# akvas/grates

Hardware: AMD Instinct MI355X
Metric: d/o-96 solutions/s to 0.25deg grid + full-cov GFLOP/s at 1/2/4/8 MI355X (higher is better)
Workload: dtype f64; 1 GPU; batch of 240 monthly solutions d/o 96 -> 0.25 deg GeographicGrid (720x1440), kernel ewh, per GPU; max_degree=96, epochs_per_gpu=240, parallelism=epochs sharded over 1 GPU(s), no collective, fused_kernel=True, fourfold_symmetry=True, rotation_folded_kernel=True, rotations=10, settle_launches=300

## Files before the change

grates_amd/_lib.py:

```python

import ctypes
import os

_HERE = os.path.dirname(os.path.abspath(__file__))
LIB_PATH = os.path.join(_HERE, 'lib', 'libshg.so')

c_double_p = ctypes.c_void_p
c_plan_p = ctypes.c_void_p


class ShgError(RuntimeError):

    def __init__(self, function, status, message):
        super().__init__('{0} failed with status {1}: {2}'.format(function, status, message))
        self.function = function
        self.status = status


PROTOTYPES = {
    'shg_plan_create': [ctypes.POINTER(c_plan_p), ctypes.c_int, ctypes.c_int, c_double_p, c_double_p, ctypes.c_int, c_double_p, ctypes.c_int],
    'shg_plan_destroy': [c_plan_p],
    'shg_plan_set_chunk': [c_plan_p, ctypes.c_int],
    'shg_plan_set_path': [c_plan_p, ctypes.c_int],
    'shg_plan_set_rotations': [c_plan_p, ctypes.c_int],
    'shg_plan_set_stage_limit': [c_plan_p, ctypes.c_int],
    'shg_plan_set_order_pruning': [c_plan_p, ctypes.c_int],
    'shg_plan_order_cutoffs': [c_plan_p, ctypes.POINTER(ctypes.c_int), ctypes.c_int, ctypes.POINTER(ctypes.c_int), ctypes.POINTER(ctypes.c_int)],
    'shg_rot_order_cutoffs': [ctypes.c_int, ctypes.c_int, c_double_p, c_double_p, ctypes.POINTER(ctypes.c_int), ctypes.c_int, ctypes.POINTER(ctypes.c_int)],
    'shg_rot_level_tables': [ctypes.c_int, ctypes.c_int, ctypes.c_int, ctypes.c_int, ctypes.c_int, c_double_p, ctypes.POINTER(ctypes.c_int32), c_double_p,
                             ctypes.c_int64, ctypes.POINTER(ctypes.c_int32), ctypes.c_int64],
    'shg_plan_info': [c_plan_p, ctypes.POINTER(ctypes.c_int64)],
    'shg_analysis_info': [c_plan_p, c_double_p],
    'shg_plan_profile': [c_plan_p, ctypes.c_int],
    'shg_plan_profile_read': [c_plan_p, ctypes.POINTER(ctypes.c_double), ctypes.POINTER(ctypes.c_int64)],
    'shg_synthesis': [c_plan_p, c_double_p, ctypes.c_int, c_double_p, ctypes.c_void_p],
    'shg_synthesis_points': [ctypes.c_int, c_double_p, c_double_p, c_double_p, ctypes.c_int, c_double_p, ctypes.c_int, c_double_p, ctypes.c_void_p],
    'shg_legendre': [ctypes.c_int, c_double_p, ctypes.c_int, c_double_p, ctypes.c_void_p],
    'shg_legendre_order': [ctypes.c_int, ctypes.c_int, c_double_p, ctypes.c_int, c_double_p, ctypes.c_void_p],
    'shg_trigonometric': [ctypes.c_int, c_double_p, ctypes.c_int, c_double_p, ctypes.c_void_p],
    'shg_synthesis_matrix_order': [ctypes.c_int, ctypes.c_int, ctypes.c_int, c_double_p, ctypes.c_int, c_double_p, ctypes.c_int, c_double_p, ctypes.c_int,
                                   c_double_p, c_double_p, ctypes.c_void_p],
# ... 138 lines not shown
```

grates_amd/csrc/common.h:

```cpp
#pragma once

#include <hip/hip_runtime.h>

#include <algorithm>
#include <atomic>
#include <cstdarg>
#include <cstdint>
#include <cstdio>
#include <cstdlib>
#include <mutex>
#include <vector>

#include "../../include/shg.h"

namespace shg {

int fail(int code, const char* fmt, ...);
int zero_fill(double* p, long long ld, long long cols, long long rows, hipStream_t stream);
int zero_fill(int* p, hipStream_t stream);
int triangle_copy(int n, const double* src, int ld, long long stride, int batch, double* dst, bool upper, hipStream_t stream);
enum ScratchSlot { kScratchSplitK = 0, kScratchAnaFold = 1, kScratchAnaTransform = 2, kScratchAnaSolution = 3, kScratchAnaFlag = 4,
                   kScratchSeriesIn = 5, kScratchSeriesOut = 6 ,
                   kScratchTriangle = 7 ,
                   kScratchBlocks = 8  };
// ... 207 lines not shown
constexpr int kRotPruneMaxDegree = 128;
constexpr int kEpochTile = 8;
constexpr int kLatTile = 64;

}

struct shg_plan {
    int device = 0;
    int N = 0, nlat = 0, nlon = 0;
    int ldlat = 0;
    bool sym4 = false;
    int rotR = 0;
    std::vector<double> lon_host;
    shg::DeviceArray<double> rot_trig;
    bool order_pruning = true;
    std::vector<int> rot_levels;
    std::vector<int> rot_level_set;
    std::vector<int> rot_trig_piece;
    std::vector<int> rot_item_rec, rot_item_nrec, rot_item_ntrip;
    shg::DeviceArray<int> rot_levtab_d;
    bool rot_levtab_valid = false;
    bool sym_ns = false;
    int ngroups = 1;
    int goff[5] = {0, 0, 0, 0, 0};
    int K = 0;
    int ncol = 0;
    int ncoltiles = 0;
    int chunk = 16;

    shg::DeviceArray<double> ct;
// ... 119 lines not shown
```

grates_amd/csrc/plan.hip:

```cpp
#include <cmath>
#include <cstring>
#include <string>

#include <map>
#include <memory>
#include <mutex>
#include <utility>
#include <vector>

#include "common.h"

namespace shg {

static thread_local std::string g_last_error;

int fail(int code, const char* fmt, ...) {
    char buf[512];
    va_list ap;
    va_start(ap, fmt);
    vsnprintf(buf, sizeof(buf), fmt, ap);
    va_end(ap);
    g_last_error = buf;
    return code;
}
// ... 478 lines not shown

extern "C" int shg_plan_set_stage_limit(shg_plan* p, int limit) {
    SHG_REQUIRE(p != nullptr, "shg_plan_set_stage_limit: NULL plan");
    std::unique_lock<std::mutex> lock(p->mtx);
    return rot_set_stage_limit(p, limit);
}

extern "C" int shg_plan_set_order_pruning(shg_plan* p, int enable) {
    SHG_REQUIRE(p != nullptr, "shg_plan_set_order_pruning: NULL plan");
    SHG_REQUIRE(enable == 0 || enable == 1, "shg_plan_set_order_pruning: %d not in {0, 1}", enable);
    std::unique_lock<std::mutex> lock(p->mtx);
    p->order_pruning = enable != 0;
    return SHG_OK;
}

extern "C" int shg_plan_order_cutoffs(const shg_plan* p, int* levels, int capacity, int* nblocks, int* enabled) {
    SHG_REQUIRE(p != nullptr && nblocks != nullptr, "shg_plan_order_cutoffs: NULL argument");
    SHG_REQUIRE(capacity >= 0 && (levels != nullptr || capacity == 0), "shg_plan_order_cutoffs: NULL table of %d entries", capacity);
    const bool applies = rot_applicable(p) && !p->rot_levels.empty();
    *nblocks = applies ? (int)p->rot_levels.size() : 0;
    if (enabled) *enabled = applies && p->order_pruning ? 1 : 0;
    for (int i = 0; i < *nblocks && i < capacity; ++i) levels[i] = p->rot_levels[i];
    return SHG_OK;
}

extern "C" int shg_rot_order_cutoffs(int N, int nlat, const double* colat_h, const double* kn_h, int* levels, int capacity, int* nblocks) {
    SHG_REQUIRE(N >= 1 && N <= kRotPruneMaxDegree, "shg_rot_order_cutoffs: degree %d out of range [1, %d]", N, kRotPruneMaxDegree);
    SHG_REQUIRE(nlat > 0 && colat_h && kn_h && nblocks, "shg_rot_order_cutoffs: NULL or empty table");
    SHG_REQUIRE(capacity >= 0 && (levels != nullptr || capacity == 0), "shg_rot_order_cutoffs: NULL table of %d entries", capacity);
    std::vector<int> badmap, lv;
// ... 55 lines not shown
        return fail(SHG_ERR_UNSUPPORTED, "shg_plan_set_rotations: the panel of %d rotations at degree %d does not fit the LDS", want, p->N);
    }
    SHG_HIP(hipDeviceSynchronize());
    if (rot_applicable(p)) {
        const int rc = build_rot_trig(p, p->lon_host.data());
        if (rc) return rc;
    }
    return SHG_OK;
}

extern "C" int shg_plan_info(const shg_plan* p, int64_t which[8]) {
    SHG_REQUIRE(p != nullptr && which != nullptr, "shg_plan_info: NULL argument");
    which[0] = p->N;
    which[1] = p->nlat;
    which[2] = p->nlon;
    which[3] = (p->sym4 ? 1 : 0) | (p->sym_ns ? 2 : 0) | (rot_applicable(p) ? 4 : 0);
    which[4] = p->chunk;
    which[5] = p->K;
    which[6] = (p->path >= 2 || (p->path == 0 && (rot_applicable(p) || fused_chunk_for(p) != 0 || fused32_applicable(p)))) ? 1 : 0;
    which[7] = p->path | (rot_applicable(p) ? p->rotR << 8 : 0);
    return SHG_OK;
}
```

grates_amd/csrc/synthesis_rot.hip:

```cpp
#include <algorithm>
#include <cmath>
#include <cstdlib>

#include "common.h"

#ifndef SHG_STORE_AUX
#define SHG_STORE_AUX 2
#endif

namespace shg {

typedef double double4_t __attribute__((ext_vector_type(4)));
typedef double double2_t __attribute__((ext_vector_type(2)));
typedef unsigned int uint4_t __attribute__((ext_vector_type(4)));

#ifndef SHG_ROT_PREFERENCE
#define SHG_ROT_PREFERENCE 10, 9, 6, 3
#endif
#ifndef SHG_ROT_WAVES
#define SHG_ROT_WAVES 8
#endif
#ifndef SHG_RING_DEPTH
#define SHG_RING_DEPTH (SHG_ROT_WAVES > 8 ? 3 : 5)
#endif
// ... 2 lines not shown
constexpr int kRingDepth = SHG_RING_DEPTH;
constexpr int kRingSlots = kRingDepth + 1;
constexpr int kRingDoubles = kWaves * kRingSlots * 128;
constexpr int kMaxClasses = kRotMaxClasses;

template <int R>
struct RotTraits {
    static constexpr int kClasses = R / 2 + 1, kTwo = R % 2 == 0 ? 2 : 1, kAcc = 2 * R;
    static constexpr int acc_of(int r) { return r == 0 ? 0 : (R % 2 == 0 && 2 * r == R) ? 2 : 2 * kTwo + 4 * (r - 1); }
};

struct RotParams {
    int N, nlat, nlon, B, nit, nh;
    int nd;
    int nct;
    int npieces;
    int cls_nk[kMaxClasses];
    int cls_cnt[kMaxClasses];
    int nslot;
#ifdef SHG_EXPERIMENT
    int dbg;
    int stagger;
    int stagger2;
#endif
    int Qtot;
    const double* cpk4;
    const double* pkf;
    const int4* itemtab;
    int nrec, ntrip;
    int* sem;
// ... 37 lines not shown

__device__ __forceinline__ void store_b64_soff(double v, int4_s rsrc, unsigned voff, unsigned soff) {
    asm volatile("s_mov_b32 m0, %3\n\ts_nop 0\n\tbuffer_store_dwordx2 %0, %1, %2, m0 offen nt"
                 :
                 : "v"(v), "v"(voff), "s"(rsrc), "s"(soff)
                 : "memory");
}

template <int N>
__device__ __forceinline__ void wait_vmcnt() {
    asm volatile("s_waitcnt vmcnt(%0)" ::"i"(N) : "memory");
    __builtin_amdgcn_sched_barrier(0);
}

template <int R>
__device__ __forceinline__ void rot_images(double4_t* acc, int r);

template <>
__device__ __forceinline__ void rot_images<6>(double4_t* acc, int r) {
    constexpr double g = 0.86602540378443864676;
    const double ca0 = acc[0][r], sb0 = acc[1][r], ca3 = acc[2][r], sb3 = acc[3][r];
    const double ca1 = acc[4][r], sa1 = acc[5][r], cb1 = acc[6][r], sb1 = acc[7][r];
    const double ca2 = acc[8][r], sa2 = acc[9][r], cb2 = acc[10][r], sb2 = acc[11][r];
#pragma unroll
    for (int sgn = 0; sgn < 2; ++sgn) {
        const double x0 = sgn ? ca0 - sb0 : ca0 + sb0, x3 = sgn ? ca3 - sb3 : ca3 + sb3;
        const double x1 = sgn ? ca1 - sb1 : ca1 + sb1, y1 = sgn ? cb1 + sa1 : cb1 - sa1;
        const double x2 = sgn ? ca2 - sb2 : ca2 + sb2, y2 = sgn ? cb2 + sa2 : cb2 - sa2;
        const double t = fma(-0.5, x2, x0);
        const double e0 = x0 + x2, e1 = fma(g, y2, t), e2 = fma(-g, y2, t);
        const double u = fma(0.5, x1, -x3);
        const double o0 = x1 + x3, o1 = fma(g, y1, u), o2 = fma(g, y1, -u);
        acc[6 * sgn + 0][r] = e0 + o0;
        acc[6 * sgn + 3][r] = e0 - o0;
        acc[6 * sgn + 1][r] = e1 + o1;
        acc[6 * sgn + 4][r] = e1 - o1;
        acc[6 * sgn + 2][r] = e2 + o2;
        acc[6 * sgn + 5][r] = e2 - o2;
    }
}

template <>
__device__ __forceinline__ void rot_images<3>(double4_t* acc, int r) {
    constexpr double g = 0.86602540378443864676;
    const double ca0 = acc[0][r], sb0 = acc[1][r];
    const double ca1 = acc[2][r], sa1 = acc[3][r], cb1 = acc[4][r], sb1 = acc[5][r];
#pragma unroll
    for (int sgn = 0; sgn < 2; ++sgn) {
        const double x0 = sgn ? ca0 - sb0 : ca0 + sb0;
        const double x1 = sgn ? ca1 - sb1 : ca1 + sb1, y1 = sgn ? cb1 + sa1 : cb1 - sa1;
        const double t = fma(-0.5, x1, x0);
        acc[3 * sgn + 0][r] = x0 + x1;
        acc[3 * sgn + 1][r] = fma(g, y1, t);
        acc[3 * sgn + 2][r] = fma(-g, y1, t);
    }
}

template <>
__device__ __forceinline__ void rot_images<9>(double4_t* acc, int r) {
    constexpr double c1 = 0.76604444311897803520, c2 = 0.17364817766693034885, c4 = -0.93969262078590838405;
    constexpr double s1 = 0.64278760968653932632, s2 = 0.98480775301220805937, s3 = 0.86602540378443864676, s4 = 0.34202014332566873304;
    const double ca0 = acc[0][r], sb0 = acc[1][r];
    double ca[4], sa[4], cb[4], sb[4];
#pragma unroll
    for (int j = 0; j < 4; ++j) {
        ca[j] = acc[2 + 4 * j][r];
        sa[j] = acc[3 + 4 * j][r];
        cb[j] = acc[4 + 4 * j][r];
        sb[j] = acc[5 + 4 * j][r];
    }
#pragma unroll
    for (int sgn = 0; sgn < 2; ++sgn) {
        const double x0 = sgn ? ca0 - sb0 : ca0 + sb0;
        double x[4], y[4];
#pragma unroll
        for (int j = 0; j < 4; ++j) {
            x[j] = sgn ? ca[j] - sb[j] : ca[j] + sb[j];
            y[j] = sgn ? cb[j] + sa[j] : cb[j] - sa[j];
        }
        const double x1 = x[0], x2 = x[1], x3 = x[2], x4 = x[3], y1 = y[0], y2 = y[1], y3 = y[2], y4 = y[3];
        const double t = (x1 + x2) + x4, x03 = x0 + x3;
        const double h = fma(-0.5, x3, x0), u = s3 * y3;
        const double C1 = fma(c1, x1, fma(c2, x2, fma(c4, x4, h)));
        const double C2 = fma(c2, x1, fma(c4, x2, fma(c1, x4, h)));
        const double C3 = fma(-0.5, t, x03);
        const double C4 = fma(c4, x1, fma(c1, x2, fma(c2, x4, h)));
        const double S1 = fma(s1, y1, fma(s2, y2, fma(s4, y4, u)));
        const double S2 = fma(s2, y1, fma(s4, y2, fma(-s1, y4, -u)));
        const double S3 = s3 * ((y1 - y2) + y4);
        const double S4 = fma(s4, y1, fma(-s1, y2, fma(-s2, y4, u)));
        acc[9 * sgn + 0][r] = x03 + t;
        acc[9 * sgn + 1][r] = C1 + S1;
        acc[9 * sgn + 8][r] = C1 - S1;
        acc[9 * sgn + 2][r] = C2 + S2;
        acc[9 * sgn + 7][r] = C2 - S2;
        acc[9 * sgn + 3][r] = C3 + S3;
        acc[9 * sgn + 6][r] = C3 - S3;
        acc[9 * sgn + 4][r] = C4 + S4;
        acc[9 * sgn + 5][r] = C4 - S4;
    }
}

template <>
__device__ __forceinline__ void rot_images<10>(double4_t* acc, int r) {
    constexpr double c1 = 0.80901699437494742410, c2 = 0.30901699437494742410;
    constexpr double s1 = 0.58778525229247312917, s2 = 0.95105651629515357212;
    const double ca0 = acc[0][r], sb0 = acc[1][r], ca5 = acc[2][r], sb5 = acc[3][r];
    double ca[4], sa[4], cb[4], sb[4];
#pragma unroll
    for (int j = 0; j < 4; ++j) {
        ca[j] = acc[4 + 4 * j][r];
        sa[j] = acc[5 + 4 * j][r];
        cb[j] = acc[6 + 4 * j][r];
        sb[j] = acc[7 + 4 * j][r];
    }
#pragma unroll
    for (int sgn = 0; sgn < 2; ++sgn) {
        const double x0 = sgn ? ca0 - sb0 : ca0 + sb0, x5 = sgn ? ca5 - sb5 : ca5 + sb5;
        double x[4], y[4];
#pragma unroll
        for (int j = 0; j < 4; ++j) {
            x[j] = sgn ? ca[j] - sb[j] : ca[j] + sb[j];
            y[j] = sgn ? cb[j] + sa[j] : cb[j] - sa[j];
        }
        const double x1 = x[0], x2 = x[1], x3 = x[2], x4 = x[3], y1 = y[0], y2 = y[1], y3 = y[2], y4 = y[3];
        const double e0 = (x0 + x2) + x4;
        const double a1 = fma(c2, x2, fma(-c1, x4, x0)), b1 = fma(s2, y2, s1 * y4);
        const double a2 = fma(-c1, x2, fma(c2, x4, x0)), b2 = fma(s1, y2, -(s2 * y4));
        const double e1 = a1 + b1, e4 = a1 - b1, e2 = a2 + b2, e3 = a2 - b2;
        const double o0 = (x1 + x3) + x5;
        const double p = fma(c1, x1, fma(-c2, x3, -x5)), q = fma(s1, y1, s2 * y3);
        const double u = fma(c2, x1, fma(-c1, x3, x5)), v = fma(s2, y1, -(s1 * y3));
        const double o1 = q + p, o4 = q - p, o2 = v + u, o3 = v - u;
        acc[10 * sgn + 0][r] = e0 + o0;
        acc[10 * sgn + 5][r] = e0 - o0;
        acc[10 * sgn + 1][r] = e1 + o1;
        acc[10 * sgn + 6][r] = e1 - o1;
        acc[10 * sgn + 2][r] = e2 + o2;
        acc[10 * sgn + 7][r] = e2 - o2;
        acc[10 * sgn + 3][r] = e3 + o3;
        acc[10 * sgn + 8][r] = e3 - o3;
        acc[10 * sgn + 4][r] = e4 + o4;
        acc[10 * sgn + 9][r] = e4 - o4;
    }
}

struct RotStream {
    const double* iptr;
    const double* ibase;
    const double* ifirst;
    const double* ilast;
    int irem;
    unsigned im0, ring_lds;
    int cslot, pf;
    double2_t tx, abx;
};

constexpr int EP = 4;
__device__ __forceinline__ void rot_stream_init(RotStream& S, const RotParams& P, const double* As, int wave) {
    const unsigned lds0 = (unsigned)(size_t)(__attribute__((address_space(3))) const void*)As;
    S.ring_lds = lds0 + (unsigned)wave * (kRingSlots * 1024);
    S.im0 = S.ring_lds;
    const int ct0 = min(wave / EP, P.nct - 1);
    const int nq = (P.nct - ct0 + kColStride - 1) / kColStride;
    S.ifirst = P.trig + (size_t)ct0 * P.npieces * 128;
    S.ilast = S.ifirst + (size_t)(nq - 1) * kColStride * P.npieces * 128;
    S.ibase = S.ifirst;
    S.iptr = S.ifirst;
    S.irem = P.npieces;
    S.cslot = 0;
    S.pf = 0;
    S.tx = (double2_t){0.0, 0.0};
    S.abx = (double2_t){0.0, 0.0};
}

__device__ __forceinline__ void rot_issue_piece(RotStream& S, const RotParams& P, unsigned lane_off) {
    glds16(S.iptr, lane_off, S.im0);
#if defined(SHG_ROT_X) && (SHG_ROT_X & 1)
    return;
// ... 50 lines not shown
    acc[A0] = __builtin_amdgcn_mfma_f64_16x16x4f64(AB_.x, T_.x, acc[A0], 0, 0, 0);                        \
    ROT_PRIO(2);                                                                                          \
    acc[A0 + 1] = __builtin_amdgcn_mfma_f64_16x16x4f64(AB_.x, T_.y, acc[A0 + 1], 0, 0, 0);                \
    acc[A0 + 2] = __builtin_amdgcn_mfma_f64_16x16x4f64(AB_.y, T_.x, acc[A0 + 2], 0, 0, 0);                \
    acc[A0 + 3] = __builtin_amdgcn_mfma_f64_16x16x4f64(AB_.y, T_.y, acc[A0 + 3], 0, 0, 0);                \
    ROT_PRIO(0)
#define ROT_MFMA2_FIRST(A0, T_, AB_)                                                                      \
    acc[A0] = (A0) == 0 ? __builtin_amdgcn_mfma_f64_16x16x4f64(AB_.x, T_.x, acc[A0], 0, 0, 0)              \
                        : __builtin_amdgcn_mfma_f64_16x16x4f64(AB_.x, T_.x, kZero4, 0, 0, 0);             \
    acc[A0 + 1] = __builtin_amdgcn_mfma_f64_16x16x4f64(AB_.y, T_.y, kZero4, 0, 0, 0)
#define ROT_MFMA4_FIRST(A0, T_, AB_)                                                                      \
    acc[A0] = __builtin_amdgcn_mfma_f64_16x16x4f64(AB_.x, T_.x, kZero4, 0, 0, 0);                         \
    acc[A0 + 1] = __builtin_amdgcn_mfma_f64_16x16x4f64(AB_.x, T_.y, kZero4, 0, 0, 0);                     \
    acc[A0 + 2] = __builtin_amdgcn_mfma_f64_16x16x4f64(AB_.y, T_.x, kZero4, 0, 0, 0);                     \
    acc[A0 + 3] = __builtin_amdgcn_mfma_f64_16x16x4f64(AB_.y, T_.y, kZero4, 0, 0, 0)
#define ROT_CLASS(C, MF, A0, NACC)                                                                        \
    {                                                                                                     \
        const int nk_ = P.cls_nk[C];                                                                      \
        int i_ = 0;                                                                                       \
        if (nk_ >= 2) {                                                                                   \
            ROT_FETCH(ty, aby);                                                                           \
            MF##_FIRST(A0, tx, abx);                                                                      \
            ROT_FETCH(tx, abx);                                                                           \
            MF(A0, ty, aby);                                                                              \
            i_ = 2;                                                                                       \
        } else if (nk_ == 1) {                                                                            \
            ROT_FETCH(ty, aby);                                                                           \
            MF##_FIRST(A0, tx, abx);                                                                      \
            tx = ty;                                                                                      \
            abx = aby;                                                                                    \
            i_ = 1;                                                                                       \
        } else {                                                                                          \
            _Pragma("unroll") for (int z_ = ((A0) == 0 ? 1 : 0); z_ < (NACC); ++z_) acc[(A0) + z_] = kZero4; \
        }                                                                                                 \
        for (; i_ + 2 <= nk_; i_ += 2) {                                                                  \
            ROT_FETCH(ty, aby);                                                                           \
            MF(A0, tx, abx);                                                                              \
            ROT_FETCH(tx, abx);                                                                           \
            MF(A0, ty, aby);                                                                              \
        }                                                                                                 \
        if (i_ < nk_) {                                                                                   \
            ROT_FETCH(ty, aby);                                                                           \
            MF(A0, tx, abx);                                                                              \
            tx = ty;                                                                                      \
            abx = aby;                                                                                    \
        }                                                                                                 \
    }
    const double4_t kZero4 = {0.0, 0.0, 0.0, 0.0};
    double2_t tx = S.tx, abx = S.abx, ty = {0.0, 0.0}, aby = {0.0, 0.0};
    const int ct0 = wave / EP;
    for (int ct = ct0, q = 0; ct < P.nct; ct += kColStride, ++q) {
        (void)q;
        double4_t acc[T::kAcc];
        {
            const double2_t* z = panel + P.nslot * PR + rt * 16 + fk;
#pragma unroll
            for (int r = 0; r < 4; ++r) acc[0][r] = z[4 * r].x;
        }
#pragma unroll
        for (int c = 0; c < T::kClasses; ++c) {
            if (c < T::kTwo) {
                ROT_CLASS(c, ROT_MFMA2, 2 * c, 2)
            } else {
                ROT_CLASS(c, ROT_MFMA4, 2 * T::kTwo + 4 * (c - T::kTwo), 4)
            }
        }
// ... 19 lines not shown
                int w = n2 + k * nR - (ascending ? 0 : P.nd);
                w = w >= P.nlon ? w - P.nlon : w;
                const int soff = (ascending ? w + 16 * ct : w + P.nd - 16 * ct - 16) * 8;
                double a_lo, a_hi, b_lo, b_hi;
                pair_exchange(acc[t][0], acc[t][2], 0xAAAAAAAAAAAAAAAAull, a_lo, a_hi);
                pair_exchange(acc[t][1], acc[t][3], 0xAAAAAAAAAAAAAAAAull, b_lo, b_hi);
                const double2_t va = ascending ? (double2_t){a_lo, a_hi} : (double2_t){a_hi, a_lo};
                const double2_t vb = ascending ? (double2_t){b_lo, b_hi} : (double2_t){b_hi, b_lo};
                const unsigned lane_col = (ascending ? asc : desc) + (unsigned)soff;
                __builtin_amdgcn_raw_buffer_store_b128(__builtin_bit_cast(uint4_t, va), rsrc, row_a + lane_col, 0, SHG_STORE_AUX);
                __builtin_amdgcn_raw_buffer_store_b128(__builtin_bit_cast(uint4_t, vb), rsrc, row_b + lane_col, 0, SHG_STORE_AUX);
            }
        }
        ROT_STAMP(4 + 2 * min(q, 3));
    }
    S.tx = tx;
    S.abx = abx;
#undef ROT_CLASS
#undef ROT_MFMA2
#undef ROT_MFMA4
#undef ROT_MFMA2_FIRST
#undef ROT_MFMA4_FIRST
#undef ROT_FETCH
}

__device__ __forceinline__ void panel_put(double2_t* panel, int index, double2_t v) { panel[index] = v; }

template <bool NS, typename PanelPtr>
__device__ __forceinline__ void rot_phase1(const RotParams& P, PanelPtr panel, const int4* recs_wave, int bt, int it, int lane) {
    const int fr = lane & 15, fk = lane >> 4;
    constexpr int ASTRIDE = NS ? 128 : 64;
    typedef int int4_v __attribute__((ext_vector_type(4)));
    typedef const int4_v __attribute__((address_space(4))) crec_t;
// ... 175 lines not shown
        if (tid == 0) legendre_token_acquire(P.sem, P.sem_limit);
        __syncthreads();
    }
    if (!SHG_DBG(P, 2)) rot_phase1<NS>(P, panel, P.itemtab + (size_t)wave * P.nrec, bt, it, lane);
    ROT_STAMP(1);
    __syncthreads();
    if (P.sem_limit > 0 && tid == 0) legendre_token_release(P.sem);
    ROT_STAMP(2);
#ifdef SHG_EXPERIMENT
    if (P.stagger2 > 0 && wave >= EP) {
        const long long t0 = wall_clock64();
        for (int i = 0; i < 100000 && (long long)wall_clock64() - t0 < P.stagger2; ++i) __builtin_amdgcn_s_sleep(4);
    }
#endif

    if (wave / EP < P.nct && !SHG_DBG(P, 4)) {
        const double2_t* const ringp = reinterpret_cast<const double2_t*>(As) + wave * (kRingSlots * 64) + lane;
        rot_issue_piece(S, P, (unsigned)lane * 16u);
        wait_vmcnt<kRingDepth>();
        S.tx = ringp[0];
        S.cslot = 1;
        S.abx = panel[(wave % EP) * 16 + fr + fk * PR];
        S.pf = P.npieces > 1 ? 1 : 0;
        rot_phase2<NS, R>(P, As, panel, S, wave, lane, bt * 4, it);
        wait_vmcnt<4 * R>();
    } else {
        wait_vmcnt<0>();
    }
    ROT_STAMP(12);
}



static inline void order_class(int R, int m, int& cls, int& sign) {
    const int rho = m % R;
    const int r = 2 * rho <= R ? rho : R - rho;
    sign = 2 * rho <= R ? 1 : -1;
    if (R % 2 == 0)
        cls = r == 0 ? 0 : 2 * r == R ? 1 : r + 1;
    else
// ... 96 lines not shown
                const double arg = (double)m * lon_h[nlon / 2 + c];
                double* dst = &tab[(((size_t)ct * npieces + ks) * 64 + l) * 2];
                dst[0] = std::cos(arg);
                dst[1] = sg * std::sin(arg);
            }
}

int build_rot_trig(shg_plan* p, const double* lon_h) {
    const std::vector<int> full(1, p->N);
    const std::vector<int>& levels = p->rot_level_set.empty() ? full : p->rot_level_set;
    std::vector<double> all, tab;
    p->rot_trig_piece.clear();
    for (int level : levels) {
        rot_trig_stream(p->rotR, p->N, level, p->nlon, lon_h, tab);
        p->rot_trig_piece.push_back((int)(all.size() / 128));
        all.insert(all.end(), tab.begin(), tab.end());
    }
    p->rot_levtab_valid = false;
    return upload(p->rot_trig, all);
}

constexpr double kRotPruneTau = 1e-30;
constexpr int kRotLevelStep = 10;

void rot_order_cutoffs(int N, int nlat, const double* colat, const double* kn, bool ns, std::vector<int>& levels) {
    const int nh = nlat / 2;
    const int nit = ns ? ceil_div(nh, 8) : ceil_div(nlat, 16);
    levels.assign(nit, 0);
    std::vector<double> a, b, big(N + 1);
    recursion_tables(N, a, b);
// ... 86 lines not shown
    int rc = build_pkf_table(p, ns, R, stream);
    if (rc) return rc;
    const int nbt = ceil_div(B, 4);
    const int nit = ns ? ceil_div(p->nlat / 2, 8) : ceil_div(p->nlat, 16);
    rc = pack_coefficients_fused(p, ns, R, anm, B, stream);
    if (rc) return rc;
    RotParams P;
    P.N = p->N;
    P.nlat = p->nlat;
    P.nlon = p->nlon;
    P.B = B;
    P.nit = nit;
    P.nh = p->nlat / 2;
    P.nd = p->nlon / (2 * R);
    P.nct = ceil_div(P.nd, 16);
    P.nslot = rot_layout(R, p->N, P.cls_nk, P.cls_cnt, nullptr);
    P.npieces = P.nslot / 4;
#ifdef SHG_EXPERIMENT
    P.dbg = experiment_switches();
    P.stagger = getenv("SHG_STAGGER") ? atoi(getenv("SHG_STAGGER")) : 0;
    P.stagger2 = getenv("SHG_STAGGER2") ? atoi(getenv("SHG_STAGGER2")) : 0;
#endif
    P.Qtot = p->Qtot;
    P.cpk4 = p->cpk4.get();
    P.pkf = p->pkf.get();
    P.itemtab = reinterpret_cast<const int4*>(p->itemtab_d.get());
    P.nrec = p->itemtab_nrec;
    P.ntrip = p->itemtab_ntrip;
    P.sem = p->sem_d.get();
    P.sem_limit = p->sem_d ? p->stage_limit : 0;
// ... 51 lines not shown
```

grates_amd/engine.py:

```python

import ctypes
import hashlib

import numpy as np

from . import _lib


def _torch():
    import torch
    return torch


def require_gpu():
    torch = _torch()
    if not torch.cuda.is_available():
        raise RuntimeError('grates_amd: no GPU visible -- the hot path runs on MI355X only (there is no CPU fallback)')
    _lib.load()
    return torch


def device(index=None):
    torch = require_gpu()
    return torch.device('cuda', torch.cuda.current_device() if index is None else index)
# ... 45 lines not shown
        if handle is not None and handle.value:
            try:
                _lib.load().shg_plan_destroy(handle)
            except Exception:
                pass
            self._handle = None

    def info(self):
        arr = (ctypes.c_int64 * 8)()
        _lib.call('shg_plan_info', self._handle, arr)
        nblocks, enabled = ctypes.c_int(0), ctypes.c_int(0)
        _lib.call('shg_plan_order_cutoffs', self._handle, None, 0, ctypes.byref(nblocks), ctypes.byref(enabled))
        levels = (ctypes.c_int * max(nblocks.value, 1))()
        _lib.call('shg_plan_order_cutoffs', self._handle, levels, nblocks.value, ctypes.byref(nblocks), ctypes.byref(enabled))
        return {'max_degree': arr[0], 'nlat': arr[1], 'nlon': arr[2], 'fourfold_symmetry': bool(arr[3] & 1), 'north_south_symmetry': bool(arr[3] & 2),
                'rotation_symmetry': bool(arr[3] & 4), 'epochs_per_pass': arr[4], 'k_slots': arr[5], 'fused': bool(arr[6]), 'path': int(arr[7]) & 0xff, 'rotations': int(arr[7]) >> 8,
                'order_pruning': bool(enabled.value), 'order_cutoffs': [int(levels[i]) for i in range(nblocks.value)]}

    def set_path(self, path):
        _lib.call('shg_plan_set_path', self._handle, {'auto': 0, 'staged': 1, 'fused': 2, 'fused32': 5, 'rot': 6}[path])

    def set_stage_limit(self, limit):
        _lib.call('shg_plan_set_stage_limit', self._handle, int(limit))

    def set_order_pruning(self, enable):
        _lib.call('shg_plan_set_order_pruning', self._handle, 1 if enable else 0)

    def set_rotations(self, R):
        _lib.call('shg_plan_set_rotations', self._handle, int(R))

    def set_chunk(self, epochs_per_pass):
        _lib.call('shg_plan_set_chunk', self._handle, int(epochs_per_pass))

    PROFILE_KINDS = ('pack_coefficients', 'legendre_stage', 'lon_stage', 'covprop', 'analysis_lon', 'analysis_solve', 'k6', 'k7')

    def profile(self, enable=True, kinds=None):
        if enable and kinds:
            mask = 0
            for name in kinds:
                mask |= 1 << (self.PROFILE_KINDS.index(name) + 1)
            _lib.call('shg_plan_profile', self._handle, mask)
# ... 1163 lines not shown
```

include/shg.h:

```cpp
#ifndef SHG_H
#define SHG_H

#include <stdint.h>

#ifdef __cplusplus
extern "C" {
#endif

typedef struct shg_plan shg_plan;

typedef enum {
    SHG_OK = 0,
    SHG_ERR_INVALID = -1,
    SHG_ERR_HIP = -2,
    SHG_ERR_NOMEM = -3,
    SHG_ERR_UNSUPPORTED = -4
} shg_status;

int shg_plan_create(shg_plan** out, int N, int nlat, const double* colat_h, const double* kn_h,
                    int nlon, const double* lon_h, int device);
int shg_plan_destroy(shg_plan* plan);

int shg_plan_set_chunk(shg_plan* plan, int epochs_per_pass);

int shg_plan_set_path(shg_plan* plan, int path);

int shg_plan_set_stage_limit(shg_plan* plan, int limit);

int shg_plan_set_rotations(shg_plan* plan, int R);

int shg_plan_set_order_pruning(shg_plan* plan, int enable);
int shg_plan_order_cutoffs(const shg_plan* plan, int* levels, int capacity, int* nblocks, int* enabled);
int shg_rot_order_cutoffs(int N, int nlat, const double* colat_h, const double* kn_h, int* levels, int capacity, int* nblocks);
int shg_rot_level_tables(int R, int N, int level, int ns, int nlon, const double* lon_h, int32_t header[24], double* trig,
                         int64_t trig_capacity, int32_t* items, int64_t items_capacity);

int shg_plan_info(const shg_plan* plan, int64_t which[8]);

#define SHG_PROFILE_KINDS 8
int shg_plan_profile(shg_plan* plan, int enable);
int shg_plan_profile_read(shg_plan* plan, double ms[SHG_PROFILE_KINDS], int64_t launches[SHG_PROFILE_KINDS]);

int shg_synthesis(shg_plan* plan, const double* anm, int B, double* grid, void* stream);

int shg_synthesis_points(int N, const double* colat, const double* lon, const double* kn, int npts,
                         const double* anm, int B, double* values, void* stream);

int shg_epoch_rms(const double* values, int B, long long M, int accumulate, long long count, double* acc, void* stream);

int shg_legendre(int N, const double* colat, int k, double* pnm, void* stream);
// ... 163 lines not shown
```

Before: 476,600 solutions/s.

## Split half-filled last longitude tile into quarter units across waves

When the per-rotation longitude count leaves a half-filled final 16-column tile, that tile is handled by a separate quarter-tile pass. The pass uses its own accumulators and a half-row swap to form the images, and the work is spread over waves to balance load. The trig stream for the tail tile is duplicated on the host so the extra waves can stream it. The rotation butterflies are refactored into shared rot_half helpers. This adds code complexity and register pressure in exchange for less padded MFMA work and better wave balance.

```diff
diff --git a/grates_amd/_lib.py b/grates_amd/_lib.py
--- a/grates_amd/_lib.py
+++ b/grates_amd/_lib.py
@@ -25,6 +25,7 @@
     'shg_plan_set_rotations': [c_plan_p, ctypes.c_int],
     'shg_plan_set_stage_limit': [c_plan_p, ctypes.c_int],
     'shg_plan_set_order_pruning': [c_plan_p, ctypes.c_int],
+    'shg_plan_set_tail_split': [c_plan_p, ctypes.c_int],
     'shg_plan_order_cutoffs': [c_plan_p, ctypes.POINTER(ctypes.c_int), ctypes.c_int, ctypes.POINTER(ctypes.c_int), ctypes.POINTER(ctypes.c_int)],
     'shg_rot_order_cutoffs': [ctypes.c_int, ctypes.c_int, c_double_p, c_double_p, ctypes.POINTER(ctypes.c_int), ctypes.c_int, ctypes.POINTER(ctypes.c_int)],
     'shg_rot_level_tables': [ctypes.c_int, ctypes.c_int, ctypes.c_int, ctypes.c_int, ctypes.c_int, c_double_p, ctypes.POINTER(ctypes.c_int32), c_double_p,
diff --git a/grates_amd/csrc/common.h b/grates_amd/csrc/common.h
--- a/grates_amd/csrc/common.h
+++ b/grates_amd/csrc/common.h
@@ -245,6 +245,7 @@
     std::vector<double> lon_host;
     shg::DeviceArray<double> rot_trig;
     bool order_pruning = true;
+    bool tail_split = true;
     std::vector<int> rot_levels;
     std::vector<int> rot_level_set;
     std::vector<int> rot_trig_piece;
diff --git a/grates_amd/csrc/plan.hip b/grates_amd/csrc/plan.hip
--- a/grates_amd/csrc/plan.hip
+++ b/grates_amd/csrc/plan.hip
@@ -516,6 +516,14 @@
     return SHG_OK;
 }
 
+extern "C" int shg_plan_set_tail_split(shg_plan* p, int enable) {
+    SHG_REQUIRE(p != nullptr, "shg_plan_set_tail_split: NULL plan");
+    SHG_REQUIRE(enable == 0 || enable == 1, "shg_plan_set_tail_split: %d not in {0, 1}", enable);
+    std::unique_lock<std::mutex> lock(p->mtx);
+    p->tail_split = enable != 0;
+    return SHG_OK;
+}
+
 extern "C" int shg_plan_order_cutoffs(const shg_plan* p, int* levels, int capacity, int* nblocks, int* enabled) {
     SHG_REQUIRE(p != nullptr && nblocks != nullptr, "shg_plan_order_cutoffs: NULL argument");
     SHG_REQUIRE(capacity >= 0 && (levels != nullptr || capacity == 0), "shg_plan_order_cutoffs: NULL table of %d entries", capacity);
@@ -601,7 +609,7 @@
     which[0] = p->N;
     which[1] = p->nlat;
     which[2] = p->nlon;
-    which[3] = (p->sym4 ? 1 : 0) | (p->sym_ns ? 2 : 0) | (rot_applicable(p) ? 4 : 0);
+    which[3] = (p->sym4 ? 1 : 0) | (p->sym_ns ? 2 : 0) | (rot_applicable(p) ? 4 : 0) | (rot_applicable(p) && p->tail_split ? 8 : 0);
     which[4] = p->chunk;
     which[5] = p->K;
     which[6] = (p->path >= 2 || (p->path == 0 && (rot_applicable(p) || fused_chunk_for(p) != 0 || fused32_applicable(p)))) ? 1 : 0;
diff --git a/grates_amd/csrc/synthesis_rot.hip b/grates_amd/csrc/synthesis_rot.hip
--- a/grates_amd/csrc/synthesis_rot.hip
+++ b/grates_amd/csrc/synthesis_rot.hip
@@ -40,6 +40,7 @@
     int N, nlat, nlon, B, nit, nh;
     int nd;
     int nct;
+    int tail;
     int npieces;
     int cls_nk[kMaxClasses];
     int cls_cnt[kMaxClasses];
@@ -107,134 +108,108 @@
 }
 
 template <int R>
-__device__ __forceinline__ void rot_images(double4_t* acc, int r);
+__device__ __forceinline__ void rot_half(const double* x, const double* y, double* f);
 
 template <>
-__device__ __forceinline__ void rot_images<6>(double4_t* acc, int r) {
+__device__ __forceinline__ void rot_half<6>(const double* x, const double* y, double* f) {
     constexpr double g = 0.86602540378443864676;
-    const double ca0 = acc[0][r], sb0 = acc[1][r], ca3 = acc[2][r], sb3 = acc[3][r];
-    const double ca1 = acc[4][r], sa1 = acc[5][r], cb1 = acc[6][r], sb1 = acc[7][r];
-    const double ca2 = acc[8][r], sa2 = acc[9][r], cb2 = acc[10][r], sb2 = acc[11][r];
-#pragma unroll
-    for (int sgn = 0; sgn < 2; ++sgn) {
-        const double x0 = sgn ? ca0 - sb0 : ca0 + sb0, x3 = sgn ? ca3 - sb3 : ca3 + sb3;
-        const double x1 = sgn ? ca1 - sb1 : ca1 + sb1, y1 = sgn ? cb1 + sa1 : cb1 - sa1;
-        const double x2 = sgn ? ca2 - sb2 : ca2 + sb2, y2 = sgn ? cb2 + sa2 : cb2 - sa2;
-        const double t = fma(-0.5, x2, x0);
-        const double e0 = x0 + x2, e1 = fma(g, y2, t), e2 = fma(-g, y2, t);
-        const double u = fma(0.5, x1, -x3);
-        const double o0 = x1 + x3, o1 = fma(g, y1, u), o2 = fma(g, y1, -u);
-        acc[6 * sgn + 0][r] = e0 + o0;
-        acc[6 * sgn + 3][r] = e0 - o0;
-        acc[6 * sgn + 1][r] = e1 + o1;
-        acc[6 * sgn + 4][r] = e1 - o1;
-        acc[6 * sgn + 2][r] = e2 + o2;
-        acc[6 * sgn + 5][r] = e2 - o2;
-    }
+    const double x0 = x[0], x3 = x[1], x1 = x[2], y1 = y[2], x2 = x[3], y2 = y[3];
+    const double t = fma(-0.5, x2, x0);
+    const double e0 = x0 + x2, e1 = fma(g, y2, t), e2 = fma(-g, y2, t);
+    const double u = fma(0.5, x1, -x3);
+    const double o0 = x1 + x3, o1 = fma(g, y1, u), o2 = fma(g, y1, -u);
+    f[0] = e0 + o0;
+    f[3] = e0 - o0;
+    f[1] = e1 + o1;
+    f[4] = e1 - o1;
+    f[2] = e2 + o2;
+    f[5] = e2 - o2;
 }
 
 template <>
-__device__ __forceinline__ void rot_images<3>(double4_t* acc, int r) {
+__device__ __forceinline__ void rot_half<3>(const double* x, const double* y, double* f) {
     constexpr double g = 0.86602540378443864676;
-    const double ca0 = acc[0][r], sb0 = acc[1][r];
-    const double ca1 = acc[2][r], sa1 = acc[3][r], cb1 = acc[4][r], sb1 = acc[5][r];
-#pragma unroll
-    for (int sgn = 0; sgn < 2; ++sgn) {
-        const double x0 = sgn ? ca0 - sb0 : ca0 + sb0;
-        const double x1 = sgn ? ca1 - sb1 : ca1 + sb1, y1 = sgn ? cb1 + sa1 : cb1 - sa1;
-        const double t = fma(-0.5, x1, x0);
-        acc[3 * sgn + 0][r] = x0 + x1;
-        acc[3 * sgn + 1][r] = fma(g, y1, t);
-        acc[3 * sgn + 2][r] = fma(-g, y1, t);
-    }
+    const double x0 = x[0], x1 = x[1], y1 = y[1];
+    const double t = fma(-0.5, x1, x0);
+    f[0] = x0 + x1;
+    f[1] = fma(g, y1, t);
+    f[2] = fma(-g, y1, t);
 }
 
 template <>
-__device__ __forceinline__ void rot_images<9>(double4_t* acc, int r) {
+__device__ __forceinline__ void rot_half<9>(const double* x, const double* y, double* f) {
     constexpr double c1 = 0.76604444311897803520, c2 = 0.17364817766693034885, c4 = -0.93969262078590838405;
     constexpr double s1 = 0.64278760968653932632, s2 = 0.98480775301220805937, s3 = 0.86602540378443864676, s4 = 0.34202014332566873304;
-    const double ca0 = acc[0][r], sb0 = acc[1][r];
-    double ca[4], sa[4], cb[4], sb[4];
-#pragma unroll
-    for (int j = 0; j < 4; ++j) {
-        ca[j] = acc[2 + 4 * j][r];
-        sa[j] = acc[3 + 4 * j][r];
-        cb[j] = acc[4 + 4 * j][r];
-        sb[j] = acc[5 + 4 * j][r];
-    }
-#pragma unroll
-    for (int sgn = 0; sgn < 2; ++sgn) {
-        const double x0 = sgn ? ca0 - sb0 : ca0 + sb0;
-        double x[4], y[4];
-#pragma unroll
-        for (int j = 0; j < 4; ++j) {
-            x[j] = sgn ? ca[j] - sb[j] : ca[j] + sb[j];
-            y[j] = sgn ? cb[j] + sa[j] : cb[j] - sa[j];
-        }
-        const double x1 = x[0], x2 = x[1], x3 = x[2], x4 = x[3], y1 = y[0], y2 = y[1], y3 = y[2], y4 = y[3];
-        const double t = (x1 + x2) + x4, x03 = x0 + x3;
-        const double h = fma(-0.5, x3, x0), u = s3 * y3;
-        const double C1 = fma(c1, x1, fma(c2, x2, fma(c4, x4, h)));
-        const double C2 = fma(c2, x1, fma(c4, x2, fma(c1, x4, h)));
-        const double C3 = fma(-0.5, t, x03);
-        const double C4 = fma(c4, x1, fma(c1, x2, fma(c2, x4, h)));
-        const double S1 = fma(s1, y1, fma(s2, y2, fma(s4, y4, u)));
-        const double S2 = fma(s2, y1, fma(s4, y2, fma(-s1, y4, -u)));
-        const double S3 = s3 * ((y1 - y2) + y4);
-        const double S4 = fma(s4, y1, fma(-s1, y2, fma(-s2, y4, u)));
-        acc[9 * sgn + 0][r] = x03 + t;
-        acc[9 * sgn + 1][r] = C1 + S1;
-        acc[9 * sgn + 8][r] = C1 - S1;
-        acc[9 * sgn + 2][r] = C2 + S2;
-        acc[9 * sgn + 7][r] = C2 - S2;
-        acc[9 * sgn + 3][r] = C3 + S3;
-        acc[9 * sgn + 6][r] = C3 - S3;
-        acc[9 * sgn + 4][r] = C4 + S4;
-        acc[9 * sgn + 5][r] = C4 - S4;
-    }
+    const double x0 = x[0], x1 = x[1], x2 = x[2], x3 = x[3], x4 = x[4], y1 = y[1], y2 = y[2], y3 = y[3], y4 = y[4];
+    const double t = (x1 + x2) + x4, x03 = x0 + x3;
+    const double h = fma(-0.5, x3, x0), u = s3 * y3;
+    const double C1 = fma(c1, x1, fma(c2, x2, fma(c4, x4, h)));
+    const double C2 = fma(c2, x1, fma(c4, x2, fma(c1, x4, h)));
+    const double C3 = fma(-0.5, t, x03);
+    const double C4 = fma(c4, x1, fma(c1, x2, fma(c2, x4, h)));
+    const double S1 = fma(s1, y1, fma(s2, y2, fma(s4, y4, u)));
+    const double S2 = fma(s2, y1, fma(s4, y2, fma(-s1, y4, -u)));
+    const double S3 = s3 * ((y1 - y2) + y4);
+    const double S4 = fma(s4, y1, fma(-s1, y2, fma(-s2, y4, u)));
+    f[0] = x03 + t;
+    f[1] = C1 + S1;
+    f[8] = C1 - S1;
+    f[2] = C2 + S2;
+    f[7] = C2 - S2;
+    f[3] = C3 + S3;
+    f[6] = C3 - S3;
+    f[4] = C4 + S4;
+    f[5] = C4 - S4;
 }
 
 template <>
-__device__ __forceinline__ void rot_images<10>(double4_t* acc, int r) {
+__device__ __forceinline__ void rot_half<10>(const double* x, const double* y, double* f) {
     constexpr double c1 = 0.80901699437494742410, c2 = 0.30901699437494742410;
     constexpr double s1 = 0.58778525229247312917, s2 = 0.95105651629515357212;
-    const double ca0 = acc[0][r], sb0 = acc[1][r], ca5 = acc[2][r], sb5 = acc[3][r];
-    double ca[4], sa[4], cb[4], sb[4];
-#pragma unroll
-    for (int j = 0; j < 4; ++j) {
-        ca[j] = acc[4 + 4 * j][r];
-        sa[j] = acc[5 + 4 * j][r];
-        cb[j] = acc[6 + 4 * j][r];
-        sb[j] = acc[7 + 4 * j][r];
-    }
+    const double x0 = x[0], x5 = x[1], x1 = x[2], x2 = x[3], x3 = x[4], x4 = x[5], y1 = y[2], y2 = y[3], y3 = y[4], y4 = y[5];
+    const double e0 = (x0 + x2) + x4;
+    const double a1 = fma(c2, x2, fma(-c1, x4, x0)), b1 = fma(s2, y2, s1 * y4);
+    const double a2 = fma(-c1, x2, fma(c2, x4, x0)), b2 = fma(s1, y2, -(s2 * y4));
+    const double e1 = a1 + b1, e4 = a1 - b1, e2 = a2 + b2, e3 = a2 - b2;
+    const double o0 = (x1 + x3) + x5;
+    const double p = fma(c1, x1, fma(-c2, x3, -x5)), q = fma(s1, y1, s2 * y3);
+    const double u = fma(c2, x1, fma(-c1, x3, x5)), v = fma(s2, y1, -(s1 * y3));
+    const double o1 = q + p, o4 = q - p, o2 = v + u, o3 = v - u;
+    f[0] = e0 + o0;
+    f[5] = e0 - o0;
+    f[1] = e1 + o1;
+    f[6] = e1 - o1;
+    f[2] = e2 + o2;
+    f[7] = e2 - o2;
+    f[3] = e3 + o3;
+    f[8] = e3 - o3;
+    f[4] = e4 + o4;
+    f[9] = e4 - o4;
+}
+
+template <int R>
+__device__ __forceinline__ void rot_images(double4_t* acc, int r) {
+    using T = RotTraits<R>;
+    double s[T::kAcc];
+#pragma unroll
+    for (int i = 0; i < T::kAcc; ++i) s[i] = acc[i][r];
 #pragma unroll
     for (int sgn = 0; sgn < 2; ++sgn) {
-        const double x0 = sgn ? ca0 - sb0 : ca0 + sb0, x5 = sgn ? ca5 - sb5 : ca5 + sb5;
-        double x[4], y[4];
-#pragma unroll
-        for (int j = 0; j < 4; ++j) {
-            x[j] = sgn ? ca[j] - sb[j] : ca[j] + sb[j];
-            y[j] = sgn ? cb[j] + sa[j] : cb[j] - sa[j];
-        }
-        const double x1 = x[0], x2 = x[1], x3 = x[2], x4 = x[3], y1 = y[0], y2 = y[1], y3 = y[2], y4 = y[3];
-        const double e0 = (x0 + x2) + x4;
-        const double a1 = fma(c2, x2, fma(-c1, x4, x0)), b1 = fma(s2, y2, s1 * y4);
-        const double a2 = fma(-c1, x2, fma(c2, x4, x0)), b2 = fma(s1, y2, -(s2 * y4));
-        const double e1 = a1 + b1, e4 = a1 - b1, e2 = a2 + b2, e3 = a2 - b2;
-        const double o0 = (x1 + x3) + x5;
-        const double p = fma(c1, x1, fma(-c2, x3, -x5)), q = fma(s1, y1, s2 * y3);
-        const double u = fma(c2, x1, fma(-c1, x3, x5)), v = fma(s2, y1, -(s1 * y3));
-        const double o1 = q + p, o4 = q - p, o2 = v + u, o3 = v - u;
-        acc[10 * sgn + 0][r] = e0 + o0;
-        acc[10 * sgn + 5][r] = e0 - o0;
-        acc[10 * sgn + 1][r] = e1 + o1;
-        acc[10 * sgn + 6][r] = e1 - o1;
-        acc[10 * sgn + 2][r] = e2 + o2;
-        acc[10 * sgn + 7][r] = e2 - o2;
-        acc[10 * sgn + 3][r] = e3 + o3;
-        acc[10 * sgn + 8][r] = e3 - o3;
-        acc[10 * sgn + 4][r] = e4 + o4;
-        acc[10 * sgn + 9][r] = e4 - o4;
+        double x[T::kClasses], y[T::kClasses], f[R];
+#pragma unroll
+        for (int c = 0; c < T::kClasses; ++c) {
+            if (c < T::kTwo) {
+                x[c] = sgn ? s[2 * c] - s[2 * c + 1] : s[2 * c] + s[2 * c + 1];
+                y[c] = 0.0;
+            } else {
+                const int a0 = 2 * T::kTwo + 4 * (c - T::kTwo);
+                x[c] = sgn ? s[a0] - s[a0 + 3] : s[a0] + s[a0 + 3];
+                y[c] = sgn ? s[a0 + 2] + s[a0 + 1] : s[a0 + 2] - s[a0 + 1];
+            }
+        }
+        rot_half<R>(x, y, f);
+#pragma unroll
+        for (int k = 0; k < R; ++k) acc[R * sgn + k][r] = f[k];
     }
 }
 
@@ -250,12 +225,32 @@
 };
 
 constexpr int EP = 4;
+
+struct RotUnits {
+    int nfull, nquart, h0;
+};
+__device__ __forceinline__ RotUnits rot_wave_units(const RotParams& P, int wave) {
+    const int g = wave / EP;
+    const int nctf = P.tail ? P.nct - 1 : P.nct;
+    RotUnits u;
+    u.nfull = g < nctf ? (nctf - g + kColStride - 1) / kColStride : 0;
+    u.nquart = 0;
+    u.h0 = 0;
+    if (P.tail) {
+        const bool odd = (P.nct & 1) != 0;
+        u.nquart = odd ? (g < 2 ? 1 : 0) : (g == 1 ? 2 : 0);
+        u.h0 = odd ? g : 0;
+    }
+    return u;
+}
+
 __device__ __forceinline__ void rot_stream_init(RotStream& S, const RotParams& P, const double* As, int wave) {
     const unsigned lds0 = (unsigned)(size_t)(__attribute__((address_space(3))) const void*)As;
     S.ring_lds = lds0 + (unsigned)wave * (kRingSlots * 1024);
     S.im0 = S.ring_lds;
+    const RotUnits u = rot_wave_units(P, wave);
     const int ct0 = min(wave / EP, P.nct - 1);
-    const int nq = (P.nct - ct0 + kColStride - 1) / kColStride;
+    const int nq = max(u.nfull + u.nquart, 1);
     S.ifirst = P.trig + (size_t)ct0 * P.npieces * 128;
     S.ilast = S.ifirst + (size_t)(nq - 1) * kColStride * P.npieces * 128;
     S.ibase = S.ifirst;
@@ -336,42 +331,44 @@
     acc[A0 + 1] = __builtin_amdgcn_mfma_f64_16x16x4f64(AB_.x, T_.y, kZero4, 0, 0, 0);                     \
     acc[A0 + 2] = __builtin_amdgcn_mfma_f64_16x16x4f64(AB_.y, T_.x, kZero4, 0, 0, 0);                     \
     acc[A0 + 3] = __builtin_amdgcn_mfma_f64_16x16x4f64(AB_.y, T_.y, kZero4, 0, 0, 0)
-#define ROT_CLASS(C, MF, A0, NACC)                                                                        \
+#define ROT_CLASS_G(C, MF, A0, NACC, FETCH, ACC, tx, abx, ty, aby)                                        \
     {                                                                                                     \
         const int nk_ = P.cls_nk[C];                                                                      \
         int i_ = 0;                                                                                       \
         if (nk_ >= 2) {                                                                                   \
-            ROT_FETCH(ty, aby);                                                                           \
+            FETCH(ty, aby);                                                                               \
             MF##_FIRST(A0, tx, abx);                                                                      \
-            ROT_FETCH(tx, abx);                                                                           \
+            FETCH(tx, abx);                                                                               \
             MF(A0, ty, aby);                                                                              \
             i_ = 2;                                                                                       \
         } else if (nk_ == 1) {                                                                            \
-            ROT_FETCH(ty, aby);                                                                           \
+            FETCH(ty, aby);                                                                               \
             MF##_FIRST(A0, tx, abx);                                                                      \
             tx = ty;                                                                                      \
             abx = aby;                                                                                    \
             i_ = 1;                                                                                       \
         } else {                                                                                          \
-            _Pragma("unroll") for (int z_ = ((A0) == 0 ? 1 : 0); z_ < (NACC); ++z_) acc[(A0) + z_] = kZero4; \
+            _Pragma("unroll") for (int z_ = ((A0) == 0 ? 1 : 0); z_ < (NACC); ++z_) ACC[(A0) + z_] = kZero4;\
         }                                                                                                 \
         for (; i_ + 2 <= nk_; i_ += 2) {                                                                  \
-            ROT_FETCH(ty, aby);                                                                           \
+            FETCH(ty, aby);                                                                               \
             MF(A0, tx, abx);                                                                              \
-            ROT_FETCH(tx, abx);                                                                           \
+            FETCH(tx, abx);                                                                               \
             MF(A0, ty, aby);                                                                              \
         }                                                                                                 \
         if (i_ < nk_) {                                                                                   \
-            ROT_FETCH(ty, aby);                                                                           \
+            FETCH(ty, aby);                                                                               \
             MF(A0, tx, abx);                                                                              \
             tx = ty;                                                                                      \
             abx = aby;                                                                                    \
         }                                                                                                 \
     }
+#define ROT_CLASS(C, MF, A0, NACC) ROT_CLASS_G(C, MF, A0, NACC, ROT_FETCH, acc, tx, abx, ty, aby)
     const double4_t kZero4 = {0.0, 0.0, 0.0, 0.0};
     double2_t tx = S.tx, abx = S.abx, ty = {0.0, 0.0}, aby = {0.0, 0.0};
     const int ct0 = wave / EP;
-    for (int ct = ct0, q = 0; ct < P.nct; ct += kColStride, ++q) {
+    const int nctf = P.tail ? P.nct - 1 : P.nct;
+    for (int ct = ct0, q = 0; ct < nctf; ct += kColStride, ++q) {
         (void)q;
         double4_t acc[T::kAcc];
         {
@@ -421,9 +418,93 @@
         }
         ROT_STAMP(4 + 2 * min(q, 3));
     }
+
+    const double* const ringq = As + wave * (kRingSlots * 128) + 2 * (fk * 16 + (fr & 7)) + (fr >> 3);
+    const bool low = fr < 8;
+    const RotUnits units = rot_wave_units(P, wave);
+    for (int hq = 0; hq < units.nquart; ++hq) {
+        const int h = units.h0 + hq;
+        const double* const prowq = reinterpret_cast<const double*>(panel) + 2 * (rt * 16 + 8 * h + (fr & 7) + fk * PR) + (fr >> 3);
+#define ROT_FETCHQ(T_, A_)                                                                                \
+    do {                                                                                                  \
+        __builtin_amdgcn_sched_barrier(0);                                                                \
+        rot_issue_piece(S, P, lane_off);                                                                  \
+        wait_vmcnt<kRingDepth>();                                                                         \
+        T_ = ringq[S.cslot * 128];                                                                        \
+        S.cslot = S.cslot + 1 == kRingSlots ? 0 : S.cslot + 1;                                            \
+        A_ = prowq[S.pf * (8 * PR)];                                                                      \
+        S.pf = S.pf + 1 == P.npieces ? 0 : S.pf + 1;                                                      \
+        __builtin_amdgcn_sched_barrier(0);                                                                \
+    } while (0)
+#define ROT_MFMAQ(A0, T_, A_) qacc[A0] = __builtin_amdgcn_mfma_f64_16x16x4f64(A_, T_, qacc[A0], 0, 0, 0)
+#define ROT_MFMAQ_FIRST(A0, T_, A_)                                                                       \
+    qacc[A0] = (A0) == 0 ? __builtin_amdgcn_mfma_f64_16x16x4f64(A_, T_, qacc[A0], 0, 0, 0)                \
+                         : __builtin_amdgcn_mfma_f64_16x16x4f64(A_, T_, kZero4, 0, 0, 0)
+        double tqx = ringq[(S.cslot == 0 ? kRingSlots - 1 : S.cslot - 1) * 128], aqx = prowq[0], tqy = 0.0, aqy = 0.0;
+        double4_t qacc[T::kClasses];
+        {
+            const double2_t* z = panel + P.nslot * PR + rt * 16 + 8 * h + fk;
+            qacc[0] = (double4_t){low ? z[0].x : 0.0, low ? z[4].x : 0.0, 0.0, 0.0};
+        }
+#pragma unroll
+        for (int c = 0; c < T::kClasses; ++c) {
+            ROT_CLASS_G(c, ROT_MFMAQ, c, 1, ROT_FETCHQ, qacc, tqx, aqx, tqy, aqy)
+        }
+        ROT_STAMP(3 + 2 * min(units.nfull + hq, 3));
+
+        const double sg = low ? 1.0 : -1.0;
+        double img[R][2];
+#pragma unroll
+        for (int r = 0; r < 2; ++r) {
+            double x[T::kClasses], y[T::kClasses], f[R];
+#pragma unroll
+            for (int c = 0; c < T::kClasses; ++c) {
+                double a_lo = qacc[c][r], a_hi = qacc[c][r + 2];
+                asm("" : "+v"(a_lo), "+v"(a_hi));
+                const double u = low ? a_lo : a_hi;
+                x[c] = fma(sg, u, swap_half_row(u));
+                y[c] = 0.0;
+                if (c >= T::kTwo) {
+                    const double v = low ? a_hi : a_lo;
+                    y[c] = fma(-sg, swap_half_row(v), v);
+                }
+            }
+            rot_half<R>(x, y, f);
+#pragma unroll
+            for (int k = 0; k < R; ++k) img[k][r] = f[k];
+        }
+        {
+            const int b = b0 + rt;
+            const bool epoch_ok = b < P.B && !SHG_DBG(P, 1);
+            double* const Gb = P.G + (size_t)min(b, P.B - 1) * P.nlat * P.nlon;
+            const __amdgpu_buffer_rsrc_t rsrc = __builtin_amdgcn_make_buffer_rsrc(Gb, 0, grid_bytes, 0x00020000);
+            const int par = fr & 1, ce = fr & 6;
+            const int sl = 8 * h + fk + (par ? 4 : 0);
+            const unsigned row = epoch_ok && slot_valid(sl) ? (unsigned)grid_row(sl) * (unsigned)P.nlon * 8u : 0x80000000u;
+            const unsigned lane_part = row + (low ? (unsigned)(16 * (P.nct - 1) + ce) * 8u : (unsigned)(6 - ce) * 8u);
+#pragma unroll
+            for (int j = 0; j < R; ++j) {
+                const int jn = j + 1 == R ? 0 : j + 1;
+                int wa = n2 + j * nR, wd = n2 + j * nR + P.nd;
+                wa = wa >= P.nlon ? wa - P.nlon : wa;
+                wd = wd >= P.nlon ? wd - P.nlon : wd;
+                const double v0 = low ? img[j][0] : img[jn][0], v1 = low ? img[j][1] : img[jn][1];
+                double c_lo, c_hi;
+                pair_exchange(v0, v1, 0xAAAAAAAAAAAAAAAAull, c_lo, c_hi);
+                const double2_t vc = {low ? c_lo : c_hi, low ? c_hi : c_lo};
+                const unsigned lane_col = lane_part + (unsigned)((low ? wa : wd) * 8);
+                __builtin_amdgcn_raw_buffer_store_b128(__builtin_bit_cast(uint4_t, vc), rsrc, lane_col, 0, SHG_STORE_AUX);
+            }
+        }
+        ROT_STAMP(4 + 2 * min(units.nfull + hq, 3));
+#undef ROT_FETCHQ
+#undef ROT_MFMAQ
+#undef ROT_MFMAQ_FIRST
+    }
     S.tx = tx;
     S.abx = abx;
 #undef ROT_CLASS
+#undef ROT_CLASS_G
 #undef ROT_MFMA2
 #undef ROT_MFMA4
 #undef ROT_MFMA2_FIRST
@@ -629,7 +710,8 @@
     }
 #endif
 
-    if (wave / EP < P.nct && !SHG_DBG(P, 4)) {
+    const RotUnits units = rot_wave_units(P, wave);
+    if (units.nfull + units.nquart > 0 && !SHG_DBG(P, 4)) {
         const double2_t* const ringp = reinterpret_cast<const double2_t*>(As) + wave * (kRingSlots * 64) + lane;
         rot_issue_piece(S, P, (unsigned)lane * 16u);
         wait_vmcnt<kRingDepth>();
@@ -638,7 +720,10 @@
         S.abx = panel[(wave % EP) * 16 + fr + fk * PR];
         S.pf = P.npieces > 1 ? 1 : 0;
         rot_phase2<NS, R>(P, As, panel, S, wave, lane, bt * 4, it);
-        wait_vmcnt<4 * R>();
+        if (units.nquart > 0)
+            wait_vmcnt<R>();
+        else
+            wait_vmcnt<4 * R>();
     } else {
         wait_vmcnt<0>();
     }
@@ -765,6 +850,12 @@
     for (int level : levels) {
         rot_trig_stream(p->rotR, p->N, level, p->nlon, lon_h, tab);
         p->rot_trig_piece.push_back((int)(all.size() / 128));
+        const int nd = p->nlon / (2 * p->rotR), nct = ceil_div(nd, 16);
+        if (nd % 16 == 8) {
+            const size_t tile = (tab.size() / 128 - 1) / nct * 128;
+            const std::vector<double> last(tab.begin() + (size_t)(nct - 1) * tile, tab.begin() + (size_t)nct * tile);
+            for (int copy = 0; copy < 2; ++copy) tab.insert(tab.begin() + (size_t)nct * tile, last.begin(), last.end());
+        }
         all.insert(all.end(), tab.begin(), tab.end());
     }
     p->rot_levtab_valid = false;
@@ -881,6 +972,7 @@
     P.nh = p->nlat / 2;
     P.nd = p->nlon / (2 * R);
     P.nct = ceil_div(P.nd, 16);
+    P.tail = p->tail_split && P.nd % 16 == 8 && kColStride == 2 ? 1 : 0;
     P.nslot = rot_layout(R, p->N, P.cls_nk, P.cls_cnt, nullptr);
     P.npieces = P.nslot / 4;
 #ifdef SHG_EXPERIMENT
diff --git a/grates_amd/engine.py b/grates_amd/engine.py
--- a/grates_amd/engine.py
+++ b/grates_amd/engine.py
@@ -83,7 +83,7 @@
         levels = (ctypes.c_int * max(nblocks.value, 1))()
         _lib.call('shg_plan_order_cutoffs', self._handle, levels, nblocks.value, ctypes.byref(nblocks), ctypes.byref(enabled))
         return {'max_degree': arr[0], 'nlat': arr[1], 'nlon': arr[2], 'fourfold_symmetry': bool(arr[3] & 1), 'north_south_symmetry': bool(arr[3] & 2),
-                'rotation_symmetry': bool(arr[3] & 4), 'epochs_per_pass': arr[4], 'k_slots': arr[5], 'fused': bool(arr[6]), 'path': int(arr[7]) & 0xff, 'rotations': int(arr[7]) >> 8,
+                'rotation_symmetry': bool(arr[3] & 4), 'tail_split': bool(arr[3] & 8), 'epochs_per_pass': arr[4], 'k_slots': arr[5], 'fused': bool(arr[6]), 'path': int(arr[7]) & 0xff, 'rotations': int(arr[7]) >> 8,
                 'order_pruning': bool(enabled.value), 'order_cutoffs': [int(levels[i]) for i in range(nblocks.value)]}
 
     def set_path(self, path):
@@ -94,6 +94,9 @@
 
     def set_order_pruning(self, enable):
         _lib.call('shg_plan_set_order_pruning', self._handle, 1 if enable else 0)
+
+    def set_tail_split(self, enable):
+        _lib.call('shg_plan_set_tail_split', self._handle, 1 if enable else 0)
 
     def set_rotations(self, R):
         _lib.call('shg_plan_set_rotations', self._handle, int(R))
diff --git a/include/shg.h b/include/shg.h
--- a/include/shg.h
+++ b/include/shg.h
@@ -34,6 +34,8 @@
 int shg_rot_order_cutoffs(int N, int nlat, const double* colat_h, const double* kn_h, int* levels, int capacity, int* nblocks);
 int shg_rot_level_tables(int R, int N, int level, int ns, int nlon, const double* lon_h, int32_t header[24], double* trig,
                          int64_t trig_capacity, int32_t* items, int64_t items_capacity);
+
+int shg_plan_set_tail_split(shg_plan* plan, int enable);
 
 int shg_plan_info(const shg_plan* plan, int64_t which[8]);
 
```

After: 482,400 solutions/s, median of 3. No clear change (+1.2%).
